# thuanz123/enhancing-transformers

Measured on NVIDIA B200. Metric: images/sec (256x256) ViT-VQGAN fwd+bwd, higher is better.
Workload: dtype fp16 tensor-core operands / fp32 accumulate (block GEMMs and attention core), 3xtf32 (patch embed, to_pixel, pre/post_quant), fp32 (everything else)

## Files before the change

### enhancing_transformers_b200/csrc/attention_f16.cu

```cuda
#include <cstdlib>
#include "common.cuh"

namespace b200 {

namespace {

constexpr int kThreads = 608;
constexpr int kIssuerB = 18;
constexpr int kSoftmaxWarps = 16;
constexpr int DH = 64;
constexpr int kTile128 = 128 * 128;
constexpr int kTile64 = 64 * 128;
constexpr float kLog2eF = 1.4426950408889634f;
constexpr int kBoxBytes = kSoftmaxWarps * 2048;
constexpr int kFwdStages = 4;
#ifndef ATTN_DKV_STAGES
#define ATTN_DKV_STAGES 6
#endif
#ifndef ATTN_DQ_STAGES
#define ATTN_DQ_STAGES 6
#endif
constexpr int kDkvStages = ATTN_DKV_STAGES;
constexpr int kDqStages = ATTN_DQ_STAGES;

__device__ __forceinline__ void quad_bar(int q) { asm volatile("bar.sync %0, 128;" ::"r"(q + 2) : "memory"); }

__device__ __forceinline__ void umma_f16_ts(uint32_t d_tmem, uint32_t a_tmem, uint64_t bdesc, uint32_t idesc, uint32_t accumulate) {
  asm volatile(
      "{\n\t.reg .pred p;\n\tsetp.ne.b32 p, %4, 0;\n\t"
      "tcgen05.mma.cta_group::1.kind::f16 [%0], [%1], %2, %3, p;\n\t}"
      ::"r"(d_tmem), "r"(a_tmem), "l"(bdesc), "r"(idesc), "r"(accumulate) : "memory");
}
__device__ __forceinline__ void tmem_st_32x16(uint32_t taddr, const uint32_t (&r)[16]) {
  asm volatile(
      "tcgen05.st.sync.aligned.32x32b.x16.b32 [%0], "
      "{%1, %2, %3, %4, %5, %6, %7, %8, %9, %10, %11, %12, %13, %14, %15, %16};"
      ::"r"(taddr), "r"(r[0]), "r"(r[1]), "r"(r[2]), "r"(r[3]), "r"(r[4]), "r"(r[5]), "r"(r[6]), "r"(r[7]),
        "r"(r[8]), "r"(r[9]), "r"(r[10]), "r"(r[11]), "r"(r[12]), "r"(r[13]), "r"(r[14]), "r"(r[15])
      : "memory");
}
__device__ __forceinline__ void tmem_st_32x8(uint32_t taddr, const uint32_t (&r)[8]) {
  asm volatile("tcgen05.st.sync.aligned.32x32b.x8.b32 [%0], {%1, %2, %3, %4, %5, %6, %7, %8};"
               ::"r"(taddr), "r"(r[0]), "r"(r[1]), "r"(r[2]), "r"(r[3]), "r"(r[4]), "r"(r[5]), "r"(r[6]), "r"(r[7]) : "memory");
}
__device__ __forceinline__ uint32_t pack_h2(float a, float b) {
  const __half2 h = __floats2half2_rn(a, b);
  return *reinterpret_cast<const uint32_t*>(&h);
}


#ifdef B200_ATTN16_TRACE
#ifndef B200_TRACE_SKIP
#define B200_TRACE_SKIP 320
#endif
constexpr int kTraceCap = 64;
__device__ long long g_trace16[3 * 2 * kTraceCap];
#define TRACE_DECL                                                                                \
  __shared__ long long tr_buf[3][2 * kTraceCap]; int tr_n = 0;                                    \
  for (int i_ = threadIdx.x; i_ < 3 * 2 * kTraceCap; i_ += blockDim.x) (&tr_buf[0][0])[i_] = 0
#define TRACE(role, ev)                                                                           \
  do {                                                                                            \
    if (blockIdx.x == 0 && (threadIdx.x & 31) == 0) {                                             \
      const int k_ = tr_n++ - B200_TRACE_SKIP;                                                    \
      if (k_ >= 0 && k_ < kTraceCap) { tr_buf[role][2 * k_] = (ev); tr_buf[role][2 * k_ + 1] = clock64(); } \
    }                                                                                             \
  } while (0)
#define TRACE_DUMP()                                                                              \
  do {                                                                                            \
    __syncthreads();                                                                              \
    if (blockIdx.x == 0) for (int i_ = threadIdx.x; i_ < 3 * 2 * kTraceCap; i_ += blockDim.x) g_trace16[i_] = (&tr_buf[0][0])[i_]; \
  } while (0)
#else
#define TRACE_DECL
#define TRACE(role, ev) do {} while (0)
#define TRACE_DUMP() do {} while (0)
#endif

#ifndef ATTN_FWD_POLY_PAIRS
#define ATTN_FWD_POLY_PAIRS 4
#endif
#ifndef ATTN_BWD_POLY_PAIRS
#define ATTN_BWD_POLY_PAIRS 1
#endif
__device__ __forceinline__ unsigned long long f2_pack(float a, float b) {
  unsigned long long r;
  asm("mov.b64 %0, {%1, %2};" : "=l"(r) : "f"(a), "f"(b));
  return r;
}
__device__ __forceinline__ void f2_unpack(unsigned long long v, float& a, float& b) {
  asm("mov.b64 {%0, %1}, %2;" : "=f"(a), "=f"(b) : "l"(v));
}
__device__ __forceinline__ unsigned long long f2_fma(unsigned long long a, unsigned long long b, unsigned long long c) {
  unsigned long long d;
  asm("fma.rn.f32x2 %0, %1, %2, %3;" : "=l"(d) : "l"(a), "l"(b), "l"(c));
  return d;
}
__device__ __forceinline__ unsigned long long f2_add(unsigned long long a, unsigned long long b) {
  unsigned long long d;
  asm("add.rn.f32x2 %0, %1, %2;" : "=l"(d) : "l"(a), "l"(b));
  return d;
}
__device__ __forceinline__ void ex2_poly_pair(float x0, float x1, float& y0, float& y1) {
  constexpr float kMagic = 12582912.f;
// ... 499 lines not shown
        for (int i = 0; i < 64; ++i) mx = fmaxf(mx, __uint_as_float(v[i]));
        float* xs = xch + (t_it & 1) * 512 + g * 256;
        xs[hlf * 128 + row_in_tile] = mx;
        pair_bar2(bar_id);
        mx = fmaxf(mx, xs[(hlf ^ 1) * 128 + row_in_tile]);
        if (j == 0) {
          m_used = mx;
        } else {
          const bool grow = (mx - m_used) * c > kRescaleLog2;
          if (__any_sync(0xffffffffu, grow)) {
            const float m_new = grow ? mx : m_used;
            const float alpha = ex2_approx((m_used - m_new) * c);
            mbar_wait(&pv_done[g], (t_it - 1) & 1);
            tcgen05_fence_after();
#pragma unroll 1
            for (int cc = 0; cc < 32; cc += 8) {
              uint32_t ov[8];
              tmem_ld_32x8(o_addr + cc, ov);
              tmem_ld_wait();
#pragma unroll
              for (int i = 0; i < 8; ++i) ov[i] = __float_as_uint(__uint_as_float(ov[i]) * alpha);
              tmem_st_32x8(o_addr + cc, ov);
            }
            tmem_st_wait();
            l *= alpha;
            m_used = m_new;
          }
        }
        const float mc = m_used * c;
        float sum = 0.f, sum1 = 0.f;
#pragma unroll
        for (int hh = 0; hh < 2; ++hh) {
          uint32_t pk[16];
#pragma unroll
          for (int i = 0; i < 16; ++i) {
            const int e = hh * 32 + 2 * i;
            float a0, a1;
            ex2_pair(poly_slot<ATTN_FWD2_POLY_PAIRS, 32>(hh * 16 + i), fmaf(__uint_as_float(v[e]), c, -mc), fmaf(__uint_as_float(v[e + 1]), c, -mc), a0, a1);
            sum += a0; sum1 += a1;
            pk[i] = pack_half2_sat(a0, a1);
          }
          tmem_st_32x16(s_addr + hlf * 32 + hh * 16, pk);
        }
        tmem_st_wait();
        tcgen05_fence_before();
        __syncwarp();
        if (lane == 0) mbar_arrive(&p_full[g]);
        l += sum + sum1;
      }
      float* ls = xch + 1024 + g * 256;
      ls[hlf * 128 + row_in_tile] = l;
      mbar_wait(&pv_done[g], (t_it - 1) & 1);
      tcgen05_fence_after();
      uint32_t ov[32];
      tmem_ld_32x32(o_addr, ov);
      tmem_ld_wait();
      tcgen05_fence_before();
      pair_bar2(bar_id);
      l += ls[(hlf ^ 1) * 128 + row_in_tile];
      if (lane == 0) mbar_arrive(&o_free[g]);
      float r[32];
#pragma unroll
      for (int i = 0; i < 32; ++i) r[i] = __uint_as_float(ov[i]);
      const int row0 = qp * 256 + g * 128 + q * 32;
      store_box_h(obox + (warp - 2) * 2048, &tmO, r, 1.f / l, h * DH + hlf * 32, row0, b, lane);
      const int row = row0 + lane;
      if (row < p.N && hlf == 0) p.lse[((long long)b * p.heads + h) * p.N + row] = m_used * p.scale + logf(l);
      pair_bar2(bar_id);
    }
    if (lane == 0) bulk_wait_group_read<0>();
  }
  tcgen05_fence_before();
  __syncthreads();
  if (warp == 1) {
    tcgen05_fence_after();
    tmem_dealloc<1>(tmem_base, 512);
  }
}

struct BwdParams {
  const float* lse;
  const float* delta;
  float* delta_w;
  int N, heads, tiles128, sub64, total_items;
  float scale;
};

__device__ __forceinline__ uint32_t packed_a_col(int k) { return (uint32_t)(k * 16); }
constexpr int kTB = 3;
constexpr int kPArrivals = kSoftmaxWarps / 2;
constexpr uint32_t kColDP = 192, kColAcc = 384;

__global__ void __launch_bounds__(kThreads, 1)
attn_bwd_dkv_f16_kernel(const __grid_constant__ CUtensorMap tmQKV128, const __grid_constant__ CUtensorMap tmQKV64,
                        const __grid_constant__ CUtensorMap tmDO64, const __grid_constant__ CUtensorMap tmOut, const BwdParams p) {
  extern __shared__ uint8_t smem_raw[];
  uint8_t* smem = smem_align1024(smem_raw);
  constexpr int NST = kDkvStages;
  uint8_t* KVs = smem;
  uint8_t* St = smem + 4 * kTile128;
  uint8_t* obox = St + NST * 2 * kTile64;
  uint64_t* bars = reinterpret_cast<uint64_t*>(obox + kBoxBytes);
  uint64_t* kv_full = bars + 0;
  uint64_t* kv_empty = bars + 2;
  uint64_t* acc_full = bars + 4;
  uint64_t* acc_empty = bars + 5;
  uint64_t* s_full = bars + 6;
  uint64_t* p_full = bars + 9;
  uint64_t* sfree = bars + 12;
  uint64_t* qd_full = bars + 15;
  uint64_t* qd_empty = qd_full + NST;
  uint32_t* tmem_slot = reinterpret_cast<uint32_t*>(qd_full + 2 * NST);

  const int warp = threadIdx.x >> 5, lane = threadIdx.x & 31;
  TRACE_DECL;
  if (warp == 0 && lane == 0) {
    tma_prefetch_desc(&tmQKV128); tma_prefetch_desc(&tmQKV64); tma_prefetch_desc(&tmDO64);
    for (int s = 0; s < NST; ++s) { mbar_init(&qd_full[s], 1); mbar_init(&qd_empty[s], 2); }
    for (int s = 0; s < 2; ++s) { mbar_init(&kv_full[s], 1); mbar_init(&kv_empty[s], 1); }
    for (int s = 0; s < kTB; ++s) { mbar_init(&s_full[s], 1); mbar_init(&p_full[s], kPArrivals); mbar_init(&sfree[s], 1); }
    mbar_init(acc_full, 1); mbar_init(acc_empty, kSoftmaxWarps);
    fence_barrier_init();
  }
  if (warp == 1) tmem_alloc<1>(tmem_slot, 512);
  tcgen05_fence_before();
  __syncthreads();
  tcgen05_fence_after();
  const uint32_t tmem_base = *tmem_slot;
  const int inner = p.heads * DH;
  const int NS = p.sub64;

  if (warp == 0) {
    uint32_t sub_it = 0, item_it = 0;
    for (int w = blockIdx.x; w < p.total_items; w += gridDim.x, ++item_it) {
      const int kt = w % p.tiles128;
      const int bh = w / p.tiles128;
      const int h = bh % p.heads, b = bh / p.heads;
      const int ib = item_it & 1;
      mbar_wait(&kv_empty[ib], ((item_it >> 1) & 1) ^ 1);
      if (elect_one()) {
        mbar_arrive_expect_tx(&kv_full[ib], 2 * kTile128);
        tma_load_3d(KVs + ib * 2 * kTile128, &tmQKV128, &kv_full[ib], inner + h * DH, kt * 128, b);
        tma_load_3d(KVs + ib * 2 * kTile128 + kTile128, &tmQKV128, &kv_full[ib], 2 * inner + h * DH, kt * 128, b);
      }
      __syncwarp();
      for (int i = 0; i < NS; ++i, ++sub_it) {
        const int s = sub_it % NST;
        const uint32_t ph = (sub_it / NST) & 1;
        uint8_t* st = St + s * 2 * kTile64;
        mbar_wait(&qd_empty[s], ph ^ 1);
        if (elect_one()) {
          mbar_arrive_expect_tx(&qd_full[s], 2 * kTile64);
          tma_load_3d(st, &tmQKV64, &qd_full[s], h * DH, i * 64, b);
          tma_load_3d(st + kTile64, &tmDO64, &qd_full[s], h * DH, i * 64, b);
        }
        __syncwarp();
      }
    }
  } else if (warp == 1) {
    constexpr uint32_t idesc_s = make_idesc_f16(128, 64, 0, 0);
    const uint64_t kd0 = kmajor_desc(KVs);
    const uint64_t qd0 = kmajor_desc(St);
    uint32_t sd_it = 0, item_it = 0;
    for (int w = blockIdx.x; w < p.total_items; w += gridDim.x, ++item_it) {
      const int ib = item_it & 1;
      mbar_wait(&kv_full[ib], (item_it >> 1) & 1);
      const uint64_t kd = desc_advance(kd0, ib * 2 * kTile128);
      const uint64_t vd = desc_advance(kd, kTile128);
      for (int i = 0; i < NS; ++i, ++sd_it) {
        const int s = sd_it % kTB;
        const uint32_t ph = (sd_it / kTB) & 1;
        const int r = sd_it % NST;
        TRACE(0, 100);
        mbar_wait2(&qd_full[r], (sd_it / NST) & 1, &sfree[s], ph ^ 1);
        TRACE(0, 102);
        tcgen05_fence_after();
        if (elect_one()) {
          const uint64_t qd = desc_advance(qd0, r * 2 * kTile64);
          const uint64_t dd = desc_advance(qd, kTile64);
#pragma unroll
          for (int k = 0; k < DH / 16; ++k)
            umma_f16<1>(tmem_base + s * 64, desc_advance(kd, k * kKStepK), desc_advance(qd, k * kKStepK), idesc_s, k != 0);
#pragma unroll
          for (int k = 0; k < DH / 16; ++k)
            umma_f16<1>(tmem_base + kColDP + s * 64, desc_advance(vd, k * kKStepK), desc_advance(dd, k * kKStepK), idesc_s, k != 0);
          umma_commit<1>(&s_full[s]);
          umma_commit<1>(&qd_empty[r]);
          if (i == NS - 1) umma_commit<1>(&kv_empty[ib]);
        }
        __syncwarp();
        TRACE(0, 103);
      }
    }
  } else if (warp == kIssuerB) {
    constexpr uint32_t idesc_g = make_idesc_f16(128, DH, 0, 1);
    const uint64_t qm0 = mnmajor_desc(St);
    uint32_t dv_it = 0, item_it = 0;
    for (int w = blockIdx.x; w < p.total_items; w += gridDim.x, ++item_it) {
      for (int i = 0; i < NS; ++i, ++dv_it) {
        const int s = dv_it % kTB;
        const uint32_t ph = (dv_it / kTB) & 1;
        const int r = dv_it % NST;
        if (i == 0) mbar_wait(acc_empty, (item_it & 1) ^ 1);
        TRACE(1, 110);
        mbar_wait2(&qd_full[r], (dv_it / NST) & 1, &p_full[s], ph);
        TRACE(1, 111);
        tcgen05_fence_after();
        if (elect_one()) {
          const uint64_t qmd = desc_advance(qm0, r * 2 * kTile64);
          const uint64_t dmd = desc_advance(qmd, kTile64);
          const uint32_t acc_on = i > 0;
#pragma unroll
          for (int k = 0; k < 4; ++k)
            umma_f16_ts(tmem_base + kColAcc, tmem_base + s * 64 + packed_a_col(k), desc_advance(dmd, k * kKStepMN), idesc_g, acc_on | (k != 0));
#pragma unroll
          for (int k = 0; k < 4; ++k)
            umma_f16_ts(tmem_base + kColAcc + 64, tmem_base + kColDP + s * 64 + packed_a_col(k), desc_advance(qmd, k * kKStepMN), idesc_g, acc_on | (k != 0));
          umma_commit<1>(&qd_empty[r]);
          umma_commit<1>(&sfree[s]);
          if (i == NS - 1) umma_commit<1>(acc_full);
        }
        __syncwarp();
        TRACE(1, 112);
      }
    }
  } else {
    const int q = warp & 3;
    const int sub = (warp - 2) >> 2;
    const uint32_t lane_off = (uint32_t)(q * 32) << 16;
    const float c = p.scale * kLog2eF;
    float* bc = reinterpret_cast<float*>(bars + 64) + (warp - 2) * 64;
    uint32_t t_it = 0, item_it = 0;
    for (int w = blockIdx.x; w < p.total_items; w += gridDim.x, ++item_it) {
      const int kt = w % p.tiles128;
      const int bh = w / p.tiles128;
      const int h = bh % p.heads, b = bh / p.heads;
      const float* lb = p.lse + ((long long)b * p.heads + h) * p.N;
      const float* eb = p.delta + ((long long)b * p.heads + h) * p.N;
      const int grp = sub & 1, half = sub >> 1;
      const int qcol = half * 32 + lane;
      const uint32_t t_base = item_it * (uint32_t)NS;
      float rawL = 0.f, rawE = 0.f;
      bool nvalid = grp < NS && grp * 64 + qcol < p.N;
      if (nvalid) { rawL = lb[grp * 64 + qcol]; rawE = eb[grp * 64 + qcol]; }
      auto chunk = [&](const uint32_t (&v)[16], const uint32_t (&g)[16], int col, int boff) {
        uint32_t pp[8], ds[8];
#pragma unroll
        for (int j = 0; j < 4; ++j) {
          const float4 L = reinterpret_cast<const float4*>(bc + boff)[j];
          const float4 E = reinterpret_cast<const float4*>(bc + 32 + boff)[j];
          float p0, p1, p2, p3;
          ex2_pair(poly_slot<ATTN_BWD_POLY_PAIRS, 8>(2 * j), fmaf(__uint_as_float(v[4 * j]), c, -L.x), fmaf(__uint_as_float(v[4 * j + 1]), c, -L.y), p0, p1);
          ex2_pair(poly_slot<ATTN_BWD_POLY_PAIRS, 8>(2 * j + 1), fmaf(__uint_as_float(v[4 * j + 2]), c, -L.z), fmaf(__uint_as_float(v[4 * j + 3]), c, -L.w), p2, p3);
          pp[2 * j] = pack_h2(p0, p1);
          pp[2 * j + 1] = pack_h2(p2, p3);
          ds[2 * j] = pack_half2_sat(p0 * (__uint_as_float(g[4 * j]) - E.x), p1 * (__uint_as_float(g[4 * j + 1]) - E.y));
          ds[2 * j + 1] = pack_half2_sat(p2 * (__uint_as_float(g[4 * j + 2]) - E.z), p3 * (__uint_as_float(g[4 * j + 3]) - E.w));
        }
        tmem_st_32x8(tmem_base + lane_off + col, pp);
        tmem_st_32x8(tmem_base + lane_off + kColDP + col, ds);
      };
      for (int i = grp; i < NS; i += 2) {
        const uint32_t t = t_base + i;
        const int s = t % kTB;
        bc[lane] = nvalid ? rawL * kLog2eF : INFINITY;
        bc[32 + lane] = nvalid ? rawE : 0.f;
        {
          const int qi = (i + 2) * 64 + qcol;
          nvalid = i + 2 < NS && qi < p.N;
          if (nvalid) { rawL = lb[qi]; rawE = eb[qi]; }
        }
        if (warp == 2) TRACE(2, 120);
        mbar_wait(&s_full[s], (t / kTB) & 1);
        if (warp == 2) TRACE(2, 121);
        tcgen05_fence_after();
        __syncwarp();
        const int col = s * 64 + half * 32;
        uint32_t vA[16], gA[16], vB[16], gB[16];
        tmem_ld_32x16(tmem_base + lane_off + col, vA);
        tmem_ld_32x16(tmem_base + lane_off + kColDP + col, gA);
        tmem_ld_wait();
        if (warp == 2) TRACE(2, 122);
        tmem_ld_32x16(tmem_base + lane_off + col + 16, vB);
        tmem_ld_32x16(tmem_base + lane_off + kColDP + col + 16, gB);
        chunk(vA, gA, col, 0);
        tmem_ld_wait();
        chunk(vB, gB, col + 16, 16);
        if (warp == 2) TRACE(2, 123);
        tmem_st_wait();
        tcgen05_fence_before();
        __syncwarp();
        if (lane == 0) mbar_arrive(&p_full[s]);
        if (warp == 2) TRACE(2, 124);
      }
      t_it += NS;
      mbar_wait(acc_full, item_it & 1);
      tcgen05_fence_after();
      {
        uint32_t v[32];
        tmem_ld_32x32(tmem_base + lane_off + kColAcc + sub * 32, v);
        tmem_ld_wait();
        float r[32];
#pragma unroll
        for (int j = 0; j < 32; ++j) r[j] = __uint_as_float(v[j]);
        const int col0 = (sub < 2 ? 2 * inner : inner) + h * DH + (sub & 1) * 32;
        store_box_h(obox + (warp - 2) * 2048, &tmOut, r, sub < 2 ? 1.f : p.scale, col0, kt * 128 + q * 32, b, lane);
      }
      tcgen05_fence_before();
      __syncwarp();
      if (lane == 0) mbar_arrive(acc_empty);
    }
    if (lane == 0) bulk_wait_group_read<0>();
  }
  tcgen05_fence_before();
  __syncthreads();
  if (warp == 1) {
    tcgen05_fence_after();
    tmem_dealloc<1>(tmem_base, 512);
  }
#ifndef B200_ATTN16_TRACE_FWD
  TRACE_DUMP();
#endif
}

__global__ void __launch_bounds__(kThreads, 1)
attn_bwd_dq_f16_kernel(const __grid_constant__ CUtensorMap tmQKV128, const __grid_constant__ CUtensorMap tmDO128,
                       const __grid_constant__ CUtensorMap tmO128, const __grid_constant__ CUtensorMap tmQKV64,
                       const __grid_constant__ CUtensorMap tmOut16, const BwdParams p) {
  extern __shared__ uint8_t smem_raw[];
  uint8_t* smem = smem_align1024(smem_raw);
  constexpr int NST = kDqStages;
  constexpr int kItem = 3 * kTile128;
  uint8_t* QDs = smem;
  uint8_t* St = smem + 2 * kItem;
  uint8_t* obox = St + NST * 2 * kTile64;
  uint64_t* bars = reinterpret_cast<uint64_t*>(obox + kBoxBytes / 2);
  uint64_t* q_full = bars + 0;
  uint64_t* q_empty = bars + 2;
  uint64_t* acc_full = bars + 4;
  uint64_t* acc_empty = bars + 5;
  uint64_t* s_full = bars + 6;
  uint64_t* p_full = bars + 9;
  uint64_t* sfree = bars + 12;
  uint64_t* kv_full = bars + 15;
  uint64_t* kv_empty = kv_full + NST;
  uint32_t* tmem_slot = reinterpret_cast<uint32_t*>(kv_full + 2 * NST);
  float* xch = reinterpret_cast<float*>(bars + 64);

  const int warp = threadIdx.x >> 5, lane = threadIdx.x & 31;
  if (warp == 0 && lane == 0) {
    tma_prefetch_desc(&tmQKV128); tma_prefetch_desc(&tmDO128); tma_prefetch_desc(&tmO128); tma_prefetch_desc(&tmQKV64);
    for (int s = 0; s < NST; ++s) { mbar_init(&kv_full[s], 1); mbar_init(&kv_empty[s], 2); }
    for (int s = 0; s < 2; ++s) { mbar_init(&q_full[s], 1); mbar_init(&q_empty[s], 1); }
    for (int s = 0; s < kTB; ++s) { mbar_init(&s_full[s], 1); mbar_init(&p_full[s], kPArrivals); mbar_init(&sfree[s], 1); }
    mbar_init(acc_full, 1); mbar_init(acc_empty, kSoftmaxWarps);
    fence_barrier_init();
  }
  if (warp == 1) tmem_alloc<1>(tmem_slot, 512);
  tcgen05_fence_before();
  __syncthreads();
  tcgen05_fence_after();
  const uint32_t tmem_base = *tmem_slot;
  const int inner = p.heads * DH;
  const int NS = p.sub64;

  if (warp == 0) {
    uint32_t sub_it = 0, item_it = 0;
    for (int w = blockIdx.x; w < p.total_items; w += gridDim.x, ++item_it) {
      const int qt = w % p.tiles128;
      const int bh = w / p.tiles128;
      const int h = bh % p.heads, b = bh / p.heads;
      const int ib = item_it & 1;
      mbar_wait(&q_empty[ib], ((item_it >> 1) & 1) ^ 1);
      if (elect_one()) {
        mbar_arrive_expect_tx(&q_full[ib], kItem);
        tma_load_3d(QDs + ib * kItem, &tmQKV128, &q_full[ib], h * DH, qt * 128, b);
        tma_load_3d(QDs + ib * kItem + kTile128, &tmDO128, &q_full[ib], h * DH, qt * 128, b);
        tma_load_3d(QDs + ib * kItem + 2 * kTile128, &tmO128, &q_full[ib], h * DH, qt * 128, b);
      }
      __syncwarp();
      for (int i = 0; i < NS; ++i, ++sub_it) {
        const int s = sub_it % NST;
        const uint32_t ph = (sub_it / NST) & 1;
        uint8_t* st = St + s * 2 * kTile64;
        mbar_wait(&kv_empty[s], ph ^ 1);
        if (elect_one()) {
          mbar_arrive_expect_tx(&kv_full[s], 2 * kTile64);
          tma_load_3d(st, &tmQKV64, &kv_full[s], inner + h * DH, i * 64, b);
          tma_load_3d(st + kTile64, &tmQKV64, &kv_full[s], 2 * inner + h * DH, i * 64, b);
        }
        __syncwarp();
      }
    }
  } else if (warp == 1) {
    constexpr uint32_t idesc_s = make_idesc_f16(128, 64, 0, 0);
    const uint64_t qd0 = kmajor_desc(QDs);
    const uint64_t kk0 = kmajor_desc(St);
    uint32_t sd_it = 0, item_it = 0;
    for (int w = blockIdx.x; w < p.total_items; w += gridDim.x, ++item_it) {
      const int ib = item_it & 1;
      mbar_wait(&q_full[ib], (item_it >> 1) & 1);
      const uint64_t qd = desc_advance(qd0, ib * kItem);
      const uint64_t dd = desc_advance(qd, kTile128);
      for (int i = 0; i < NS; ++i, ++sd_it) {
        const int s = sd_it % kTB;
        const uint32_t ph = (sd_it / kTB) & 1;
        const int r = sd_it % NST;
        mbar_wait2(&kv_full[r], (sd_it / NST) & 1, &sfree[s], ph ^ 1);
        tcgen05_fence_after();
        if (elect_one()) {
          const uint64_t kkd = desc_advance(kk0, r * 2 * kTile64);
          const uint64_t vkd = desc_advance(kkd, kTile64);
#pragma unroll
          for (int k = 0; k < DH / 16; ++k)
            umma_f16<1>(tmem_base + s * 64, desc_advance(qd, k * kKStepK), desc_advance(kkd, k * kKStepK), idesc_s, k != 0);
#pragma unroll
          for (int k = 0; k < DH / 16; ++k)
            umma_f16<1>(tmem_base + kColDP + s * 64, desc_advance(dd, k * kKStepK), desc_advance(vkd, k * kKStepK), idesc_s, k != 0);
          umma_commit<1>(&s_full[s]);
          umma_commit<1>(&kv_empty[r]);
          if (i == NS - 1) umma_commit<1>(&q_empty[ib]);
        }
        __syncwarp();
      }
    }
  } else if (warp == kIssuerB) {
    constexpr uint32_t idesc_g = make_idesc_f16(128, DH, 0, 1);
    const uint64_t km0 = mnmajor_desc(St);
    uint32_t dq_it = 0, item_it = 0;
    for (int w = blockIdx.x; w < p.total_items; w += gridDim.x, ++item_it) {
      for (int i = 0; i < NS; ++i, ++dq_it) {
        const int s = dq_it % kTB;
        const uint32_t ph = (dq_it / kTB) & 1;
        const int r = dq_it % NST;
        if (i == 0) mbar_wait(acc_empty, (item_it & 1) ^ 1);
        mbar_wait2(&kv_full[r], (dq_it / NST) & 1, &p_full[s], ph);
        tcgen05_fence_after();
        if (elect_one()) {
          const uint64_t kmd = desc_advance(km0, r * 2 * kTile64);
          const uint32_t acc_on = i > 0;
#pragma unroll
          for (int k = 0; k < 4; ++k)
            umma_f16_ts(tmem_base + kColAcc, tmem_base + kColDP + s * 64 + packed_a_col(k), desc_advance(kmd, k * kKStepMN), idesc_g, acc_on | (k != 0));
          umma_commit<1>(&kv_empty[r]);
          umma_commit<1>(&sfree[s]);
          if (i == NS - 1) umma_commit<1>(acc_full);
        }
        __syncwarp();
      }
    }
  } else {
    const int q = warp & 3;
    const int sub = (warp - 2) >> 2;
    constexpr int OC = DH / 4;
    const uint32_t lane_off = (uint32_t)(q * 32) << 16;
    const float c = p.scale * kLog2eF;
    uint32_t t_it = 0, item_it = 0;
    for (int w = blockIdx.x; w < p.total_items; w += gridDim.x, ++item_it) {
      const int qt = w % p.tiles128;
      const int bh = w / p.tiles128;
      const int h = bh % p.heads, b = bh / p.heads;
      const int row = qt * 128 + q * 32 + lane;
      const long long sidx = ((long long)b * p.heads + h) * p.N + row;
      const float lse2 = row < p.N ? p.lse[sidx] * kLog2eF : INFINITY;
      float dl;
      {
        const int ib = item_it & 1;
        mbar_wait(&q_full[ib], (item_it >> 1) & 1);
        const int r = q * 32 + lane;
        const uint8_t* dOt = QDs + ib * kItem + kTile128 + r * 128;
        const uint8_t* Ot = dOt + kTile128;
        float acc = 0.f;
#pragma unroll
        for (int ch = 0; ch < 2; ++ch) {
          const int off = ((sub * 2 + ch) ^ (r & 7)) << 4;
          const uint4 a = *reinterpret_cast<const uint4*>(dOt + off);
          const uint4 o = *reinterpret_cast<const uint4*>(Ot + off);
          const uint32_t aw[4] = {a.x, a.y, a.z, a.w}, ow[4] = {o.x, o.y, o.z, o.w};
#pragma unroll
          for (int k = 0; k < 4; ++k) {
            const float2 fa = __half22float2(*reinterpret_cast<const __half2*>(&aw[k]));
            const float2 fo = __half22float2(*reinterpret_cast<const __half2*>(&ow[k]));
            acc = fmaf(fa.x, fo.x, acc);
            acc = fmaf(fa.y, fo.y, acc);
          }
        }
        float* xs = xch + ib * 512;
        xs[sub * 128 + r] = acc;
        quad_bar(q);
        dl = (xs[r] + xs[128 + r]) + (xs[256 + r] + xs[384 + r]);
        if (sub == 0 && row < p.N) p.delta_w[sidx] = dl;
      }
      const int grp = sub & 1, half = sub >> 1;
      const uint32_t t_base = item_it * (uint32_t)NS;
      auto chunk = [&](const uint32_t (&v)[16], const uint32_t (&g)[16], int col, int kv_left) {
        uint32_t ds[8];
#pragma unroll
        for (int j = 0; j < 8; ++j) {
          float p0, p1;
          ex2_pair(poly_slot<ATTN_BWD_POLY_PAIRS, 8>(j), fmaf(__uint_as_float(v[2 * j]), c, -lse2), fmaf(__uint_as_float(v[2 * j + 1]), c, -lse2), p0, p1);
          ds[j] = pack_half2_sat(p0 * (__uint_as_float(g[2 * j]) - dl), p1 * (__uint_as_float(g[2 * j + 1]) - dl));
        }
        if (kv_left < 16) {
#pragma unroll
          for (int j = 0; j < 8; ++j) {
            if (2 * j >= kv_left) ds[j] = 0u;
            else if (2 * j + 1 >= kv_left) ds[j] &= 0xffffu;
          }
        }
        tmem_st_32x8(tmem_base + lane_off + kColDP + col, ds);
      };
      for (int i = grp; i < NS; i += 2) {
        const uint32_t t = t_base + i;
        const int s = t % kTB;
        mbar_wait(&s_full[s], (t / kTB) & 1);
        tcgen05_fence_after();
        const int col = s * 64 + half * 32;
        const int kv_left = p.N - i * 64 - half * 32;
        uint32_t vA[16], gA[16], vB[16], gB[16];
        tmem_ld_32x16(tmem_base + lane_off + col, vA);
        tmem_ld_32x16(tmem_base + lane_off + kColDP + col, gA);
        tmem_ld_wait();
        tmem_ld_32x16(tmem_base + lane_off + col + 16, vB);
        tmem_ld_32x16(tmem_base + lane_off + kColDP + col + 16, gB);
        chunk(vA, gA, col, kv_left);
        tmem_ld_wait();
        chunk(vB, gB, col + 16, kv_left - 16);
        tmem_st_wait();
        tcgen05_fence_before();
        __syncwarp();
        if (lane == 0) mbar_arrive(&p_full[s]);
      }
      t_it += NS;
      mbar_wait(acc_full, item_it & 1);
      tcgen05_fence_after();
      {
        uint32_t v[OC];
        tmem_ld_32x16(tmem_base + lane_off + kColAcc + sub * OC, v);
        tmem_ld_wait();
        float r[OC];
#pragma unroll
        for (int j = 0; j < OC; ++j) r[j] = __uint_as_float(v[j]);
        store_box_h16(obox + (warp - 2) * 1024, &tmOut16, r, p.scale, h * DH + sub * OC, qt * 128 + q * 32, b, lane);
      }
      tcgen05_fence_before();
      __syncwarp();
      if (lane == 0) mbar_arrive(acc_empty);
    }
    if (lane == 0) bulk_wait_group_read<0>();
  }
  tcgen05_fence_before();
  __syncthreads();
  if (warp == 1) {
    tcgen05_fence_after();
    tmem_dealloc<1>(tmem_base, 512);
  }
}


int make_tile_map(CUtensorMap* out, const void* ptr, long long ld, int N, int B, int box_rows) {
  const unsigned long long dims[3] = {(unsigned long long)ld, (unsigned long long)N, (unsigned long long)B};
  const unsigned long long strides[2] = {(unsigned long long)ld * 2, (unsigned long long)N * ld * 2};
  const unsigned box[3] = {64, (unsigned)box_rows, 1};
  return make_tensor_map(out, ptr, 2, 3, dims, strides, box, 0);
}
int make_store_map(CUtensorMap* out, const void* ptr, long long ld, int N, int B, int cols) {
  const unsigned long long dims[3] = {(unsigned long long)ld, (unsigned long long)N, (unsigned long long)B};
  const unsigned long long strides[2] = {(unsigned long long)ld * 2, (unsigned long long)N * ld * 2};
  const unsigned box[3] = {(unsigned)cols, 32, 1};
  return make_tensor_map(out, ptr, 2, 3, dims, strides, box, 3);
}

int persistent_grid(int items) {
  int grid = num_sms();
  if (sm_limit() > 0 && grid > sm_limit()) grid = sm_limit();
  return grid > items ? items : grid;
}

}

int attention_f16_forward(const void* qkv, void* out, float* lse, int B, int N, int heads, int dh, float scale, cudaStream_t stream) {
  B200_CHECK_ARG(B > 0 && N > 0 && heads > 0, "attention: empty problem");
  B200_CHECK_ARG(dh == DH, "attention_f16: dim_head must be 64 (got %d); other head sizes use the tf32 core", dh);
  B200_CHECK_ARG((reinterpret_cast<uintptr_t>(qkv) & 15) == 0 && (reinterpret_cast<uintptr_t>(out) & 15) == 0,
                 "attention: qkv/out must be 16-byte aligned");
  const int inner = heads * DH;
  CUtensorMap tmQKV, tmO;
  int rc;
  if ((rc = make_tile_map(&tmQKV, qkv, 3ll * inner, N, B, 128))) return rc;
  if ((rc = make_store_map(&tmO, out, inner, N, B, 16))) return rc;
#ifndef ATTN_FWD_V2
#define ATTN_FWD_V2 1
#endif
  static const int use_v2 = [] { const char* e = getenv("B200VQ_ATTN_FWD_V2"); return e ? atoi(e) : ATTN_FWD_V2; }();
  if (use_v2) {
    if ((rc = make_store_map(&tmO, out, inner, N, B, 32))) return rc;
    Fwd2Params p2;
    p2.lse = lse; p2.N = N; p2.heads = heads;
    p2.q_pairs = (N + 255) / 256; p2.kv_tiles = (N + 127) / 128;
    p2.total_items = p2.q_pairs * heads * B;
    p2.scale = scale;
    constexpr int smem2 = (4 + 2 * kV2Stages) * kTile128 + kBoxBytes + 512 + 1536 * 4 + 1024;
    static_assert(smem2 <= 227 * 1024, "attention forward v2: shared-memory plan exceeds 227 KB");
    B200_CONFIGURE_SMEM_ONCE(attn_fwd2_f16_kernel, smem2);
    attn_fwd2_f16_kernel<<<persistent_grid(p2.total_items), kThreads2, smem2, stream>>>(tmQKV, tmO, p2);
    B200_LAUNCH_OK("attn_fwd2_f16_kernel");
    return 0;
  }
  FwdParams p;
  p.lse = lse; p.N = N; p.heads = heads;
  p.q_tiles = (N + 127) / 128; p.kv_tiles = (N + 127) / 128;
  p.total_items = p.q_tiles * heads * B;
  p.scale = scale;
  constexpr int smem = (2 + 2 * kFwdStages) * kTile128 + kBoxBytes + 512 + 1536 * 4 + 1024;
  B200_CONFIGURE_SMEM_ONCE(attn_fwd_f16_kernel, smem);
  attn_fwd_f16_kernel<<<persistent_grid(p.total_items), kThreads, smem, stream>>>(tmQKV, tmO, p);
  B200_LAUNCH_OK("attn_fwd_f16_kernel");
  return 0;
}

int attention_f16_backward(const void* qkv, const void* out, const float* lse, const void* dout, void* dqkv, float* delta, int B, int N,
                           int heads, int dh, float scale, cudaStream_t stream) {
  B200_CHECK_ARG(B > 0 && N > 0 && heads > 0, "attention: empty problem");
  B200_CHECK_ARG(dh == DH, "attention_f16: dim_head must be 64 (got %d)", dh);
  B200_CHECK_ARG((reinterpret_cast<uintptr_t>(qkv) & 15) == 0 && (reinterpret_cast<uintptr_t>(dout) & 15) == 0 &&
                     (reinterpret_cast<uintptr_t>(dqkv) & 15) == 0 && (reinterpret_cast<uintptr_t>(out) & 15) == 0,
                 "attention: qkv/out/dout/dqkv must be 16-byte aligned");
  int rc;
  const int inner = heads * DH;
  const long long ld = 3ll * inner;
  CUtensorMap tmQKV128, tmQKV64, tmDO128, tmDO64, tmO128, tmOut, tmOut16;
  if ((rc = make_tile_map(&tmQKV128, qkv, ld, N, B, 128))) return rc;
  if ((rc = make_tile_map(&tmQKV64, qkv, ld, N, B, 64))) return rc;
  if ((rc = make_tile_map(&tmDO128, dout, inner, N, B, 128))) return rc;
  if ((rc = make_tile_map(&tmDO64, dout, inner, N, B, 64))) return rc;
  if ((rc = make_tile_map(&tmO128, out, inner, N, B, 128))) return rc;
  if ((rc = make_store_map(&tmOut, dqkv, ld, N, B, 32))) return rc;
  if ((rc = make_store_map(&tmOut16, dqkv, ld, N, B, 16))) return rc;
  BwdParams p;
  p.lse = lse; p.delta = delta; p.delta_w = delta; p.N = N; p.heads = heads;
  p.tiles128 = (N + 127) / 128; p.sub64 = (N + 63) / 64;
  p.total_items = p.tiles128 * heads * B;
  p.scale = scale;
  constexpr int smem_kv = 4 * kTile128 + kDkvStages * 2 * kTile64 + kBoxBytes + 512 + kSoftmaxWarps * 256 + 1024;
  constexpr int smem_q = 6 * kTile128 + kDqStages * 2 * kTile64 + kBoxBytes / 2 + 512 + 1024 * 4 + 1024;
  static_assert(smem_kv <= 227 * 1024 && smem_q <= 227 * 1024, "attention backward: shared-memory plan exceeds 227 KB");
  B200_CONFIGURE_SMEM_ONCE(attn_bwd_dkv_f16_kernel, smem_kv);
  B200_CONFIGURE_SMEM_ONCE(attn_bwd_dq_f16_kernel, smem_q);
  const int grid = persistent_grid(p.total_items);
  attn_bwd_dq_f16_kernel<<<grid, kThreads, smem_q, stream>>>(tmQKV128, tmDO128, tmO128, tmQKV64, tmOut16, p);
  B200_LAUNCH_OK("attn_bwd_dq_f16_kernel");
  attn_bwd_dkv_f16_kernel<<<grid, kThreads, smem_kv, stream>>>(tmQKV128, tmQKV64, tmDO64, tmOut, p);
  B200_LAUNCH_OK("attn_bwd_dkv_f16_kernel");
  return 0;
}

}
```

Measured before the change: 600.6.

## Widen attention backward sub-tiles to 128 and split S/dP buffers from packed P/dS

Both attention backward kernels now stream Q/dO (or K/V) in 128-row tiles instead of 64, so each S and dP MMA is 128x128 and the gradient MMAs run 8 k-steps per tile. TMEM is repartitioned into a single S/dP region plus separate packed P/dS buffers (one for dKV, two for dQ). A new ld_done barrier lets the next S MMA start once softmax warps have read S, before they finish writing packed P/dS. The aim is fewer, larger MMAs and less per-tile barrier overhead. In exchange, pipeline stages drop from 6 to 3 because smem per stage doubles, and the S region is single-buffered.

```diff
diff --git a/enhancing_transformers_b200/csrc/attention_f16.cu b/enhancing_transformers_b200/csrc/attention_f16.cu
--- a/enhancing_transformers_b200/csrc/attention_f16.cu
+++ b/enhancing_transformers_b200/csrc/attention_f16.cu
@@ -10,15 +10,14 @@
 constexpr int kSoftmaxWarps = 16;
 constexpr int DH = 64;
 constexpr int kTile128 = 128 * 128;
-constexpr int kTile64 = 64 * 128;
 constexpr float kLog2eF = 1.4426950408889634f;
 constexpr int kBoxBytes = kSoftmaxWarps * 2048;
 constexpr int kFwdStages = 4;
 #ifndef ATTN_DKV_STAGES
-#define ATTN_DKV_STAGES 6
+#define ATTN_DKV_STAGES 3
 #endif
 #ifndef ATTN_DQ_STAGES
-#define ATTN_DQ_STAGES 6
+#define ATTN_DQ_STAGES 3
 #endif
 constexpr int kDkvStages = ATTN_DKV_STAGES;
 constexpr int kDqStages = ATTN_DQ_STAGES;
@@ -684,43 +683,44 @@
   const float* lse;
   const float* delta;
   float* delta_w;
-  int N, heads, tiles128, sub64, total_items;
+  int N, heads, tiles128, total_items;
   float scale;
 };
 
-__device__ __forceinline__ uint32_t packed_a_col(int k) { return (uint32_t)(k * 16); }
-constexpr int kTB = 3;
-constexpr int kPArrivals = kSoftmaxWarps / 2;
-constexpr uint32_t kColDP = 192, kColAcc = 384;
+constexpr uint32_t kColS = 0, kColDP = 128, kColPk = 256, kColAcc = 384;
+constexpr int kDkvPk = 1, kDqPk = 2;
+constexpr int kTile128x2 = 2 * kTile128;
 
 __global__ void __launch_bounds__(kThreads, 1)
-attn_bwd_dkv_f16_kernel(const __grid_constant__ CUtensorMap tmQKV128, const __grid_constant__ CUtensorMap tmQKV64,
-                        const __grid_constant__ CUtensorMap tmDO64, const __grid_constant__ CUtensorMap tmOut, const BwdParams p) {
+attn_bwd_dkv_f16_kernel(const __grid_constant__ CUtensorMap tmQKV128, const __grid_constant__ CUtensorMap tmDO128,
+                        const __grid_constant__ CUtensorMap tmOut, const BwdParams p) {
   extern __shared__ uint8_t smem_raw[];
   uint8_t* smem = smem_align1024(smem_raw);
   constexpr int NST = kDkvStages;
   uint8_t* KVs = smem;
   uint8_t* St = smem + 4 * kTile128;
-  uint8_t* obox = St + NST * 2 * kTile64;
+  uint8_t* obox = St + NST * kTile128x2;
   uint64_t* bars = reinterpret_cast<uint64_t*>(obox + kBoxBytes);
   uint64_t* kv_full = bars + 0;
   uint64_t* kv_empty = bars + 2;
   uint64_t* acc_full = bars + 4;
   uint64_t* acc_empty = bars + 5;
   uint64_t* s_full = bars + 6;
-  uint64_t* p_full = bars + 9;
-  uint64_t* sfree = bars + 12;
-  uint64_t* qd_full = bars + 15;
+  uint64_t* ld_done = bars + 7;
+  uint64_t* p_full = bars + 8;
+  uint64_t* pk_free = bars + 10;
+  uint64_t* qd_full = bars + 13;
   uint64_t* qd_empty = qd_full + NST;
   uint32_t* tmem_slot = reinterpret_cast<uint32_t*>(qd_full + 2 * NST);
 
   const int warp = threadIdx.x >> 5, lane = threadIdx.x & 31;
   TRACE_DECL;
   if (warp == 0 && lane == 0) {
-    tma_prefetch_desc(&tmQKV128); tma_prefetch_desc(&tmQKV64); tma_prefetch_desc(&tmDO64);
+    tma_prefetch_desc(&tmQKV128); tma_prefetch_desc(&tmDO128);
     for (int s = 0; s < NST; ++s) { mbar_init(&qd_full[s], 1); mbar_init(&qd_empty[s], 2); }
     for (int s = 0; s < 2; ++s) { mbar_init(&kv_full[s], 1); mbar_init(&kv_empty[s], 1); }
-    for (int s = 0; s < kTB; ++s) { mbar_init(&s_full[s], 1); mbar_init(&p_full[s], kPArrivals); mbar_init(&sfree[s], 1); }
+    mbar_init(s_full, 1); mbar_init(ld_done, kSoftmaxWarps);
+    for (int s = 0; s < 2; ++s) { mbar_init(&p_full[s], kSoftmaxWarps); mbar_init(&pk_free[s], 1); }
     mbar_init(acc_full, 1); mbar_init(acc_empty, kSoftmaxWarps);
     fence_barrier_init();
   }
@@ -730,7 +730,7 @@
   tcgen05_fence_after();
   const uint32_t tmem_base = *tmem_slot;
   const int inner = p.heads * DH;
-  const int NS = p.sub64;
+  const int NS = p.tiles128;
 
   if (warp == 0) {
     uint32_t sub_it = 0, item_it = 0;
@@ -749,18 +749,18 @@
       for (int i = 0; i < NS; ++i, ++sub_it) {
         const int s = sub_it % NST;
         const uint32_t ph = (sub_it / NST) & 1;
-        uint8_t* st = St + s * 2 * kTile64;
+        uint8_t* st = St + s * kTile128x2;
         mbar_wait(&qd_empty[s], ph ^ 1);
         if (elect_one()) {
-          mbar_arrive_expect_tx(&qd_full[s], 2 * kTile64);
-          tma_load_3d(st, &tmQKV64, &qd_full[s], h * DH, i * 64, b);
-          tma_load_3d(st + kTile64, &tmDO64, &qd_full[s], h * DH, i * 64, b);
+          mbar_arrive_expect_tx(&qd_full[s], kTile128x2);
+          tma_load_3d(st, &tmQKV128, &qd_full[s], h * DH, i * 128, b);
+          tma_load_3d(st + kTile128, &tmDO128, &qd_full[s], h * DH, i * 128, b);
         }
         __syncwarp();
       }
     }
   } else if (warp == 1) {
-    constexpr uint32_t idesc_s = make_idesc_f16(128, 64, 0, 0);
+    constexpr uint32_t idesc_s = make_idesc_f16(128, 128, 0, 0);
     const uint64_t kd0 = kmajor_desc(KVs);
     const uint64_t qd0 = kmajor_desc(St);
     uint32_t sd_it = 0, item_it = 0;
@@ -770,23 +770,21 @@
       const uint64_t kd = desc_advance(kd0, ib * 2 * kTile128);
       const uint64_t vd = desc_advance(kd, kTile128);
       for (int i = 0; i < NS; ++i, ++sd_it) {
-        const int s = sd_it % kTB;
-        const uint32_t ph = (sd_it / kTB) & 1;
         const int r = sd_it % NST;
         TRACE(0, 100);
-        mbar_wait2(&qd_full[r], (sd_it / NST) & 1, &sfree[s], ph ^ 1);
+        mbar_wait2(&qd_full[r], (sd_it / NST) & 1, ld_done, (sd_it & 1) ^ 1);
         TRACE(0, 102);
         tcgen05_fence_after();
         if (elect_one()) {
-          const uint64_t qd = desc_advance(qd0, r * 2 * kTile64);
-          const uint64_t dd = desc_advance(qd, kTile64);
+          const uint64_t qd = desc_advance(qd0, r * kTile128x2);
+          const uint64_t dd = desc_advance(qd, kTile128);
 #pragma unroll
           for (int k = 0; k < DH / 16; ++k)
-            umma_f16<1>(tmem_base + s * 64, desc_advance(kd, k * kKStepK), desc_advance(qd, k * kKStepK), idesc_s, k != 0);
+            umma_f16<1>(tmem_base + kColS, desc_advance(kd, k * kKStepK), desc_advance(qd, k * kKStepK), idesc_s, k != 0);
 #pragma unroll
           for (int k = 0; k < DH / 16; ++k)
-            umma_f16<1>(tmem_base + kColDP + s * 64, desc_advance(vd, k * kKStepK), desc_advance(dd, k * kKStepK), idesc_s, k != 0);
-          umma_commit<1>(&s_full[s]);
+            umma_f16<1>(tmem_base + kColDP, desc_advance(vd, k * kKStepK), desc_advance(dd, k * kKStepK), idesc_s, k != 0);
+          umma_commit<1>(s_full);
           umma_commit<1>(&qd_empty[r]);
           if (i == NS - 1) umma_commit<1>(&kv_empty[ib]);
         }
@@ -800,26 +798,26 @@
     uint32_t dv_it = 0, item_it = 0;
     for (int w = blockIdx.x; w < p.total_items; w += gridDim.x, ++item_it) {
       for (int i = 0; i < NS; ++i, ++dv_it) {
-        const int s = dv_it % kTB;
-        const uint32_t ph = (dv_it / kTB) & 1;
+        const int pb = dv_it % kDkvPk;
+        const uint32_t ph = (dv_it / kDkvPk) & 1;
         const int r = dv_it % NST;
         if (i == 0) mbar_wait(acc_empty, (item_it & 1) ^ 1);
         TRACE(1, 110);
-        mbar_wait2(&qd_full[r], (dv_it / NST) & 1, &p_full[s], ph);
+        mbar_wait2(&qd_full[r], (dv_it / NST) & 1, &p_full[pb], ph);
         TRACE(1, 111);
         tcgen05_fence_after();
         if (elect_one()) {
-          const uint64_t qmd = desc_advance(qm0, r * 2 * kTile64);
-          const uint64_t dmd = desc_advance(qmd, kTile64);
+          const uint64_t qmd = desc_advance(qm0, r * kTile128x2);
+          const uint64_t dmd = desc_advance(qmd, kTile128);
           const uint32_t acc_on = i > 0;
 #pragma unroll
-          for (int k = 0; k < 4; ++k)
-            umma_f16_ts(tmem_base + kColAcc, tmem_base + s * 64 + packed_a_col(k), desc_advance(dmd, k * kKStepMN), idesc_g, acc_on | (k != 0));
-#pragma unroll
-          for (int k = 0; k < 4; ++k)
-            umma_f16_ts(tmem_base + kColAcc + 64, tmem_base + kColDP + s * 64 + packed_a_col(k), desc_advance(qmd, k * kKStepMN), idesc_g, acc_on | (k != 0));
+          for (int k = 0; k < 8; ++k)
+            umma_f16_ts(tmem_base + kColAcc, tmem_base + kColPk + pb * 128 + k * 8, desc_advance(dmd, k * kKStepMN), idesc_g, acc_on | (k != 0));
+#pragma unroll
+          for (int k = 0; k < 8; ++k)
+            umma_f16_ts(tmem_base + kColAcc + 64, tmem_base + kColPk + pb * 128 + 64 + k * 8, desc_advance(qmd, k * kKStepMN), idesc_g, acc_on | (k != 0));
           umma_commit<1>(&qd_empty[r]);
-          umma_commit<1>(&sfree[s]);
+          umma_commit<1>(&pk_free[pb]);
           if (i == NS - 1) umma_commit<1>(acc_full);
         }
         __syncwarp();
@@ -832,21 +830,19 @@
     const uint32_t lane_off = (uint32_t)(q * 32) << 16;
     const float c = p.scale * kLog2eF;
     float* bc = reinterpret_cast<float*>(bars + 64) + (warp - 2) * 64;
-    uint32_t t_it = 0, item_it = 0;
+    uint32_t item_it = 0;
     for (int w = blockIdx.x; w < p.total_items; w += gridDim.x, ++item_it) {
       const int kt = w % p.tiles128;
       const int bh = w / p.tiles128;
       const int h = bh % p.heads, b = bh / p.heads;
       const float* lb = p.lse + ((long long)b * p.heads + h) * p.N;
       const float* eb = p.delta + ((long long)b * p.heads + h) * p.N;
-      const int grp = sub & 1, half = sub >> 1;
-      const int qcol = half * 32 + lane;
+      const int qcol = sub * 32 + lane;
       const uint32_t t_base = item_it * (uint32_t)NS;
       float rawL = 0.f, rawE = 0.f;
-      bool nvalid = grp < NS && grp * 64 + qcol < p.N;
-      if (nvalid) { rawL = lb[grp * 64 + qcol]; rawE = eb[grp * 64 + qcol]; }
-      auto chunk = [&](const uint32_t (&v)[16], const uint32_t (&g)[16], int col, int boff) {
-        uint32_t pp[8], ds[8];
+      bool nvalid = qcol < p.N;
+      if (nvalid) { rawL = lb[qcol]; rawE = eb[qcol]; }
+      auto chunk = [&](const uint32_t (&v)[16], const uint32_t (&g)[16], int boff, uint32_t (&pp)[8], uint32_t (&ds)[8]) {
 #pragma unroll
         for (int j = 0; j < 4; ++j) {
           const float4 L = reinterpret_cast<const float4*>(bc + boff)[j];
@@ -859,43 +855,51 @@
           ds[2 * j] = pack_half2_sat(p0 * (__uint_as_float(g[4 * j]) - E.x), p1 * (__uint_as_float(g[4 * j + 1]) - E.y));
           ds[2 * j + 1] = pack_half2_sat(p2 * (__uint_as_float(g[4 * j + 2]) - E.z), p3 * (__uint_as_float(g[4 * j + 3]) - E.w));
         }
-        tmem_st_32x8(tmem_base + lane_off + col, pp);
-        tmem_st_32x8(tmem_base + lane_off + kColDP + col, ds);
       };
-      for (int i = grp; i < NS; i += 2) {
+      for (int i = 0; i < NS; ++i) {
         const uint32_t t = t_base + i;
-        const int s = t % kTB;
         bc[lane] = nvalid ? rawL * kLog2eF : INFINITY;
         bc[32 + lane] = nvalid ? rawE : 0.f;
         {
-          const int qi = (i + 2) * 64 + qcol;
-          nvalid = i + 2 < NS && qi < p.N;
+          const int qi = (i + 1) * 128 + qcol;
+          nvalid = i + 1 < NS && qi < p.N;
           if (nvalid) { rawL = lb[qi]; rawE = eb[qi]; }
         }
         if (warp == 2) TRACE(2, 120);
-        mbar_wait(&s_full[s], (t / kTB) & 1);
+        mbar_wait(s_full, t & 1);
         if (warp == 2) TRACE(2, 121);
         tcgen05_fence_after();
         __syncwarp();
-        const int col = s * 64 + half * 32;
+        const uint32_t scol = kColS + sub * 32, gcol = kColDP + sub * 32;
         uint32_t vA[16], gA[16], vB[16], gB[16];
-        tmem_ld_32x16(tmem_base + lane_off + col, vA);
-        tmem_ld_32x16(tmem_base + lane_off + kColDP + col, gA);
+        tmem_ld_32x16(tmem_base + lane_off + scol, vA);
+        tmem_ld_32x16(tmem_base + lane_off + gcol, gA);
         tmem_ld_wait();
         if (warp == 2) TRACE(2, 122);
-        tmem_ld_32x16(tmem_base + lane_off + col + 16, vB);
-        tmem_ld_32x16(tmem_base + lane_off + kColDP + col + 16, gB);
-        chunk(vA, gA, col, 0);
+        tmem_ld_32x16(tmem_base + lane_off + scol + 16, vB);
+        tmem_ld_32x16(tmem_base + lane_off + gcol + 16, gB);
+        uint32_t pp[8], ds[8];
+        chunk(vA, gA, 0, pp, ds);
         tmem_ld_wait();
-        chunk(vB, gB, col + 16, 16);
+        tcgen05_fence_before();
+        __syncwarp();
+        if (lane == 0) mbar_arrive(ld_done);
+        const int pb = t % kDkvPk;
+        mbar_wait(&pk_free[pb], ((t / kDkvPk) & 1) ^ 1);
+        tcgen05_fence_after();
+        const uint32_t pcol = kColPk + pb * 128 + sub * 16;
+        tmem_st_32x8(tmem_base + lane_off + pcol, pp);
+        tmem_st_32x8(tmem_base + lane_off + pcol + 64, ds);
+        chunk(vB, gB, 16, pp, ds);
+        tmem_st_32x8(tmem_base + lane_off + pcol + 8, pp);
+        tmem_st_32x8(tmem_base + lane_off + pcol + 72, ds);
         if (warp == 2) TRACE(2, 123);
         tmem_st_wait();
         tcgen05_fence_before();
         __syncwarp();
-        if (lane == 0) mbar_arrive(&p_full[s]);
+        if (lane == 0) mbar_arrive(&p_full[pb]);
         if (warp == 2) TRACE(2, 124);
       }
-      t_it += NS;
       mbar_wait(acc_full, item_it & 1);
       tcgen05_fence_after();
       {
@@ -927,34 +931,35 @@
 
 __global__ void __launch_bounds__(kThreads, 1)
 attn_bwd_dq_f16_kernel(const __grid_constant__ CUtensorMap tmQKV128, const __grid_constant__ CUtensorMap tmDO128,
-                       const __grid_constant__ CUtensorMap tmO128, const __grid_constant__ CUtensorMap tmQKV64,
-                       const __grid_constant__ CUtensorMap tmOut16, const BwdParams p) {
+                       const __grid_constant__ CUtensorMap tmO128, const __grid_constant__ CUtensorMap tmOut16, const BwdParams p) {
   extern __shared__ uint8_t smem_raw[];
   uint8_t* smem = smem_align1024(smem_raw);
   constexpr int NST = kDqStages;
   constexpr int kItem = 3 * kTile128;
   uint8_t* QDs = smem;
   uint8_t* St = smem + 2 * kItem;
-  uint8_t* obox = St + NST * 2 * kTile64;
+  uint8_t* obox = St + NST * kTile128x2;
   uint64_t* bars = reinterpret_cast<uint64_t*>(obox + kBoxBytes / 2);
   uint64_t* q_full = bars + 0;
   uint64_t* q_empty = bars + 2;
   uint64_t* acc_full = bars + 4;
   uint64_t* acc_empty = bars + 5;
   uint64_t* s_full = bars + 6;
-  uint64_t* p_full = bars + 9;
-  uint64_t* sfree = bars + 12;
-  uint64_t* kv_full = bars + 15;
+  uint64_t* ld_done = bars + 7;
+  uint64_t* p_full = bars + 8;
+  uint64_t* pk_free = bars + 10;
+  uint64_t* kv_full = bars + 13;
   uint64_t* kv_empty = kv_full + NST;
   uint32_t* tmem_slot = reinterpret_cast<uint32_t*>(kv_full + 2 * NST);
   float* xch = reinterpret_cast<float*>(bars + 64);
 
   const int warp = threadIdx.x >> 5, lane = threadIdx.x & 31;
   if (warp == 0 && lane == 0) {
-    tma_prefetch_desc(&tmQKV128); tma_prefetch_desc(&tmDO128); tma_prefetch_desc(&tmO128); tma_prefetch_desc(&tmQKV64);
+    tma_prefetch_desc(&tmQKV128); tma_prefetch_desc(&tmDO128); tma_prefetch_desc(&tmO128);
     for (int s = 0; s < NST; ++s) { mbar_init(&kv_full[s], 1); mbar_init(&kv_empty[s], 2); }
     for (int s = 0; s < 2; ++s) { mbar_init(&q_full[s], 1); mbar_init(&q_empty[s], 1); }
-    for (int s = 0; s < kTB; ++s) { mbar_init(&s_full[s], 1); mbar_init(&p_full[s], kPArrivals); mbar_init(&sfree[s], 1); }
+    mbar_init(s_full, 1); mbar_init(ld_done, kSoftmaxWarps);
+    for (int s = 0; s < 2; ++s) { mbar_init(&p_full[s], kSoftmaxWarps); mbar_init(&pk_free[s], 1); }
     mbar_init(acc_full, 1); mbar_init(acc_empty, kSoftmaxWarps);
     fence_barrier_init();
   }
@@ -964,7 +969,7 @@
   tcgen05_fence_after();
   const uint32_t tmem_base = *tmem_slot;
   const int inner = p.heads * DH;
-  const int NS = p.sub64;
+  const int NS = p.tiles128;
 
   if (warp == 0) {
     uint32_t sub_it = 0, item_it = 0;
@@ -984,18 +989,18 @@
       for (int i = 0; i < NS; ++i, ++sub_it) {
         const int s = sub_it % NST;
         const uint32_t ph = (sub_it / NST) & 1;
-        uint8_t* st = St + s * 2 * kTile64;
+        uint8_t* st = St + s * kTile128x2;
         mbar_wait(&kv_empty[s], ph ^ 1);
         if (elect_one()) {
-          mbar_arrive_expect_tx(&kv_full[s], 2 * kTile64);
-          tma_load_3d(st, &tmQKV64, &kv_full[s], inner + h * DH, i * 64, b);
-          tma_load_3d(st + kTile64, &tmQKV64, &kv_full[s], 2 * inner + h * DH, i * 64, b);
+          mbar_arrive_expect_tx(&kv_full[s], kTile128x2);
+          tma_load_3d(st, &tmQKV128, &kv_full[s], inner + h * DH, i * 128, b);
+          tma_load_3d(st + kTile128, &tmQKV128, &kv_full[s], 2 * inner + h * DH, i * 128, b);
         }
         __syncwarp();
       }
     }
   } else if (warp == 1) {
-    constexpr uint32_t idesc_s = make_idesc_f16(128, 64, 0, 0);
+    constexpr uint32_t idesc_s = make_idesc_f16(128, 128, 0, 0);
     const uint64_t qd0 = kmajor_desc(QDs);
     const uint64_t kk0 = kmajor_desc(St);
     uint32_t sd_it = 0, item_it = 0;
@@ -1005,21 +1010,19 @@
       const uint64_t qd = desc_advance(qd0, ib * kItem);
       const uint64_t dd = desc_advance(qd, kTile128);
       for (int i = 0; i < NS; ++i, ++sd_it) {
-        const int s = sd_it % kTB;
-        const uint32_t ph = (sd_it / kTB) & 1;
         const int r = sd_it % NST;
-        mbar_wait2(&kv_full[r], (sd_it / NST) & 1, &sfree[s], ph ^ 1);
+        mbar_wait2(&kv_full[r], (sd_it / NST) & 1, ld_done, (sd_it & 1) ^ 1);
         tcgen05_fence_after();
         if (elect_one()) {
-          const uint64_t kkd = desc_advance(kk0, r * 2 * kTile64);
-          const uint64_t vkd = desc_advance(kkd, kTile64);
+          const uint64_t kkd = desc_advance(kk0, r * kTile128x2);
+          const uint64_t vkd = desc_advance(kkd, kTile128);
 #pragma unroll
           for (int k = 0; k < DH / 16; ++k)
-            umma_f16<1>(tmem_base + s * 64, desc_advance(qd, k * kKStepK), desc_advance(kkd, k * kKStepK), idesc_s, k != 0);
+            umma_f16<1>(tmem_base + kColS, desc_advance(qd, k * kKStepK), desc_advance(kkd, k * kKStepK), idesc_s, k != 0);
 #pragma unroll
           for (int k = 0; k < DH / 16; ++k)
-            umma_f16<1>(tmem_base + kColDP + s * 64, desc_advance(dd, k * kKStepK), desc_advance(vkd, k * kKStepK), idesc_s, k != 0);
-          umma_commit<1>(&s_full[s]);
+            umma_f16<1>(tmem_base + kColDP, desc_advance(dd, k * kKStepK), desc_advance(vkd, k * kKStepK), idesc_s, k != 0);
+          umma_commit<1>(s_full);
           umma_commit<1>(&kv_empty[r]);
           if (i == NS - 1) umma_commit<1>(&q_empty[ib]);
         }
@@ -1032,20 +1035,20 @@
     uint32_t dq_it = 0, item_it = 0;
     for (int w = blockIdx.x; w < p.total_items; w += gridDim.x, ++item_it) {
       for (int i = 0; i < NS; ++i, ++dq_it) {
-        const int s = dq_it % kTB;
-        const uint32_t ph = (dq_it / kTB) & 1;
+        const int pb = dq_it % kDqPk;
+        const uint32_t ph = (dq_it / kDqPk) & 1;
         const int r = dq_it % NST;
         if (i == 0) mbar_wait(acc_empty, (item_it & 1) ^ 1);
-        mbar_wait2(&kv_full[r], (dq_it / NST) & 1, &p_full[s], ph);
+        mbar_wait2(&kv_full[r], (dq_it / NST) & 1, &p_full[pb], ph);
         tcgen05_fence_after();
         if (elect_one()) {
-          const uint64_t kmd = desc_advance(km0, r * 2 * kTile64);
+          const uint64_t kmd = desc_advance(km0, r * kTile128x2);
           const uint32_t acc_on = i > 0;
 #pragma unroll
-          for (int k = 0; k < 4; ++k)
-            umma_f16_ts(tmem_base + kColAcc, tmem_base + kColDP + s * 64 + packed_a_col(k), desc_advance(kmd, k * kKStepMN), idesc_g, acc_on | (k != 0));
+          for (int k = 0; k < 8; ++k)
+            umma_f16_ts(tmem_base + kColAcc, tmem_base + kColPk + pb * 64 + k * 8, desc_advance(kmd, k * kKStepMN), idesc_g, acc_on | (k != 0));
           umma_commit<1>(&kv_empty[r]);
-          umma_commit<1>(&sfree[s]);
+          umma_commit<1>(&pk_free[pb]);
           if (i == NS - 1) umma_commit<1>(acc_full);
         }
         __syncwarp();
@@ -1057,7 +1060,7 @@
     constexpr int OC = DH / 4;
     const uint32_t lane_off = (uint32_t)(q * 32) << 16;
     const float c = p.scale * kLog2eF;
-    uint32_t t_it = 0, item_it = 0;
+    uint32_t item_it = 0;
     for (int w = blockIdx.x; w < p.total_items; w += gridDim.x, ++item_it) {
       const int qt = w % p.tiles128;
       const int bh = w / p.tiles128;
@@ -1093,10 +1096,8 @@
         dl = (xs[r] + xs[128 + r]) + (xs[256 + r] + xs[384 + r]);
         if (sub == 0 && row < p.N) p.delta_w[sidx] = dl;
       }
-      const int grp = sub & 1, half = sub >> 1;
       const uint32_t t_base = item_it * (uint32_t)NS;
-      auto chunk = [&](const uint32_t (&v)[16], const uint32_t (&g)[16], int col, int kv_left) {
-        uint32_t ds[8];
+      auto chunk = [&](const uint32_t (&v)[16], const uint32_t (&g)[16], int kv_left, uint32_t (&ds)[8]) {
 #pragma unroll
         for (int j = 0; j < 8; ++j) {
           float p0, p1;
@@ -1110,30 +1111,37 @@
             else if (2 * j + 1 >= kv_left) ds[j] &= 0xffffu;
           }
         }
-        tmem_st_32x8(tmem_base + lane_off + kColDP + col, ds);
       };
-      for (int i = grp; i < NS; i += 2) {
+      for (int i = 0; i < NS; ++i) {
         const uint32_t t = t_base + i;
-        const int s = t % kTB;
-        mbar_wait(&s_full[s], (t / kTB) & 1);
+        mbar_wait(s_full, t & 1);
         tcgen05_fence_after();
-        const int col = s * 64 + half * 32;
-        const int kv_left = p.N - i * 64 - half * 32;
+        const uint32_t scol = kColS + sub * 32, gcol = kColDP + sub * 32;
+        const int kv_left = p.N - i * 128 - sub * 32;
         uint32_t vA[16], gA[16], vB[16], gB[16];
-        tmem_ld_32x16(tmem_base + lane_off + col, vA);
-        tmem_ld_32x16(tmem_base + lane_off + kColDP + col, gA);
+        tmem_ld_32x16(tmem_base + lane_off + scol, vA);
+        tmem_ld_32x16(tmem_base + lane_off + gcol, gA);
         tmem_ld_wait();
-        tmem_ld_32x16(tmem_base + lane_off + col + 16, vB);
-        tmem_ld_32x16(tmem_base + lane_off + kColDP + col + 16, gB);
-        chunk(vA, gA, col, kv_left);
+        tmem_ld_32x16(tmem_base + lane_off + scol + 16, vB);
+        tmem_ld_32x16(tmem_base + lane_off + gcol + 16, gB);
+        uint32_t ds[8];
+        chunk(vA, gA, kv_left, ds);
         tmem_ld_wait();
-        chunk(vB, gB, col + 16, kv_left - 16);
+        tcgen05_fence_before();
+        __syncwarp();
+        if (lane == 0) mbar_arrive(ld_done);
+        const int pb = t % kDqPk;
+        mbar_wait(&pk_free[pb], ((t / kDqPk) & 1) ^ 1);
+        tcgen05_fence_after();
+        const uint32_t pcol = kColPk + pb * 64 + sub * 16;
+        tmem_st_32x8(tmem_base + lane_off + pcol, ds);
+        chunk(vB, gB, kv_left - 16, ds);
+        tmem_st_32x8(tmem_base + lane_off + pcol + 8, ds);
         tmem_st_wait();
         tcgen05_fence_before();
         __syncwarp();
-        if (lane == 0) mbar_arrive(&p_full[s]);
-      }
-      t_it += NS;
+        if (lane == 0) mbar_arrive(&p_full[pb]);
+      }
       mbar_wait(acc_full, item_it & 1);
       tcgen05_fence_after();
       {
@@ -1158,7 +1166,6 @@
     tmem_dealloc<1>(tmem_base, 512);
   }
 }
-
 
 int make_tile_map(CUtensorMap* out, const void* ptr, long long ld, int N, int B, int box_rows) {
   const unsigned long long dims[3] = {(unsigned long long)ld, (unsigned long long)N, (unsigned long long)B};
@@ -1231,28 +1238,26 @@
   int rc;
   const int inner = heads * DH;
   const long long ld = 3ll * inner;
-  CUtensorMap tmQKV128, tmQKV64, tmDO128, tmDO64, tmO128, tmOut, tmOut16;
+  CUtensorMap tmQKV128, tmDO128, tmO128, tmOut, tmOut16;
   if ((rc = make_tile_map(&tmQKV128, qkv, ld, N, B, 128))) return rc;
-  if ((rc = make_tile_map(&tmQKV64, qkv, ld, N, B, 64))) return rc;
   if ((rc = make_tile_map(&tmDO128, dout, inner, N, B, 128))) return rc;
-  if ((rc = make_tile_map(&tmDO64, dout, inner, N, B, 64))) return rc;
   if ((rc = make_tile_map(&tmO128, out, inner, N, B, 128))) return rc;
   if ((rc = make_store_map(&tmOut, dqkv, ld, N, B, 32))) return rc;
   if ((rc = make_store_map(&tmOut16, dqkv, ld, N, B, 16))) return rc;
   BwdParams p;
   p.lse = lse; p.delta = delta; p.delta_w = delta; p.N = N; p.heads = heads;
-  p.tiles128 = (N + 127) / 128; p.sub64 = (N + 63) / 64;
+  p.tiles128 = (N + 127) / 128;
   p.total_items = p.tiles128 * heads * B;
   p.scale = scale;
-  constexpr int smem_kv = 4 * kTile128 + kDkvStages * 2 * kTile64 + kBoxBytes + 512 + kSoftmaxWarps * 256 + 1024;
-  constexpr int smem_q = 6 * kTile128 + kDqStages * 2 * kTile64 + kBoxBytes / 2 + 512 + 1024 * 4 + 1024;
+  constexpr int smem_kv = 4 * kTile128 + kDkvStages * kTile128x2 + kBoxBytes + 512 + kSoftmaxWarps * 256 + 1024;
+  constexpr int smem_q = 6 * kTile128 + kDqStages * kTile128x2 + kBoxBytes / 2 + 512 + 1024 * 4 + 1024;
   static_assert(smem_kv <= 227 * 1024 && smem_q <= 227 * 1024, "attention backward: shared-memory plan exceeds 227 KB");
   B200_CONFIGURE_SMEM_ONCE(attn_bwd_dkv_f16_kernel, smem_kv);
   B200_CONFIGURE_SMEM_ONCE(attn_bwd_dq_f16_kernel, smem_q);
   const int grid = persistent_grid(p.total_items);
-  attn_bwd_dq_f16_kernel<<<grid, kThreads, smem_q, stream>>>(tmQKV128, tmDO128, tmO128, tmQKV64, tmOut16, p);
+  attn_bwd_dq_f16_kernel<<<grid, kThreads, smem_q, stream>>>(tmQKV128, tmDO128, tmO128, tmOut16, p);
   B200_LAUNCH_OK("attn_bwd_dq_f16_kernel");
-  attn_bwd_dkv_f16_kernel<<<grid, kThreads, smem_kv, stream>>>(tmQKV128, tmQKV64, tmDO64, tmOut, p);
+  attn_bwd_dkv_f16_kernel<<<grid, kThreads, smem_kv, stream>>>(tmQKV128, tmDO128, tmOut, p);
   B200_LAUNCH_OK("attn_bwd_dkv_f16_kernel");
   return 0;
 }
```

After: 601.6 (median of 6 runs). No clear change (+0.2%).
